# spla-tam/SplaTAM

Measured on AMD Instinct MI355X. Metric: track+map iters/sec @300k Gaussians (render+backward Mpix/s alongside), higher is better.
Workload: dtype f32; 1 GPU; B: 300000 Gaussians, 1200x680, SplaTAM tracking+mapping loop (2:3 mix), isotropic map; fused tracking iterations do not form dL/d(rgb, opacity, scale): the reference computes them, steps them with learning rate 0 and discards the optimizer after the frame (parameters after any number of iterations are identical); mapping iterations take their Adam step on gradients held in registers and do not sto; gaussians=300000, width=1200, height=680, views=8, sync_mode=auto, engine=fused, parallelism=1 process/GPU

## Files before the change

### splatam_amd/csrc/fused.hip

```cpp
#include "splat_device.h"

#include "fused_math.h"

namespace splat {

namespace {

constexpr int kBlock = 256;
constexpr int kFlagSum = SPLAT_ITER_SUMS - 1;

struct FusedArgs {
    SplatCamera cam;
    SplatMap map;
    SplatFrameData frame;
    SplatLossConfig cfg;
    SplatIterWorkspace ws;
    float win[11];
};

__device__ __forceinline__ int c_num_tiles(int W, int H) { return ((W + kTile - 1) / kTile) * ((H + kTile - 1) / kTile); }
__device__ __forceinline__ int c_num_groups(int W, int H) {
    return (((W + kTile - 1) / kTile + SPLAT_GROUP_TILES - 1) / SPLAT_GROUP_TILES) * (((H + kTile - 1) / kTile + SPLAT_GROUP_TILES - 1) / SPLAT_GROUP_TILES);
}

// ... 211 lines not shown
        const uint64_t key = ((uint64_t)dbits[g] << 32) | (uint32_t)i;
        for (int y = y0; y < y1; ++y)
            for (int x = x0; x < x1; ++x) {
                const unsigned tix = (unsigned)(y * c.gx + x);
                const unsigned slot = atomicAdd(&s_tile[tix], 1u);
                if (slot < stride) st.keys[(size_t)tix * stride + slot] = key;
                else spilled = true;
            }
    }
    if (spilled) st.status[1] = 1;
}

__device__ __forceinline__ double *sum_copy(double *sums) {
    const unsigned b = blockIdx.x + gridDim.x * (blockIdx.y + gridDim.y * blockIdx.z);
    return sums + (size_t)(b % SPLAT_ITER_SUM_COPIES) * SPLAT_ITER_SUMS;
}

template <int N>
__device__ __forceinline__ void block_sum_to(double *dst, const float (&v)[N], double *s_part ) {
    const int lane = threadIdx.x & 63, wave = threadIdx.x >> 6, nw = blockDim.x >> 6;
#pragma unroll
    for (int k = 0; k < N; ++k) {
        float x = v[k];
        for (int m = 32; m >= 1; m >>= 1) x += __shfl_xor(x, m, 64);
        if (lane == 0) s_part[k * nw + wave] = (double)x;
    }
    __syncthreads();
    if ((int)threadIdx.x < N) {
        double t = 0.0;
        for (int w = 0; w < nw; ++w) t += s_part[threadIdx.x * nw + w];
        if (t != 0.0) atomicAdd(dst + threadIdx.x, t);
    }
    __syncthreads();
}

__device__ __forceinline__ double sum_total(const double *sums, int k) {
    static_assert(SPLAT_ITER_SUM_COPIES == 64, "one copy per lane");
    double v = sums[(size_t)(threadIdx.x & 63) * SPLAT_ITER_SUMS + k];
    for (int m = 32; m >= 1; m >>= 1) v += __shfl_xor(v, m, 64);
    return v;
}

struct Pixel {
    bool mask;
    float d_err;
    float d_sign;
};

__device__ __forceinline__ float sgn(float x) { return (x > 0.f) ? 1.f : ((x < 0.f) ? -1.f : 0.f); }

__device__ __forceinline__ Pixel depth_pixel(const SplatLossConfig &cfg, float depth, float sil, float depth_sq, float gt, float median) {
    Pixel r;
    const float unc = depth_sq - depth * depth;
    const bool nan_ok = !(depth != depth) && !(unc != unc);
    bool m = gt > 0.f && nan_ok;
    if (cfg.ignore_outlier_depth_loss) m = m && (fabsf(gt - depth) < 10.f * median);
    if (cfg.tracking && cfg.use_sil_for_loss) m = m && (sil > cfg.sil_thres);
    r.mask = m;
    const float diff = gt - depth;
    r.d_err = m ? fabsf(diff) : 0.f;
    r.d_sign = m ? -sgn(diff) : 0.f;
    return r;
}

template <int V>
__global__ __launch_bounds__(kBlock) void track_loss_kernel(FusedArgs a, int HW) {
    __shared__ double s_part[2 * (kBlock / 64)];
    const float *o = a.ws.out6;
    float *g = a.ws.dL_dout6;
    const bool masked_im = a.cfg.use_sil_for_loss || a.cfg.ignore_outlier_depth_loss;
    const float median = a.cfg.ignore_outlier_depth_loss ? a.ws.d_cam[13] : 0.f;
    float acc[2] = {0.f, 0.f};
    const int nvec = HW / V;
    for (int i = blockIdx.x * kBlock + threadIdx.x; i < nvec; i += gridDim.x * kBlock) {
        float in[10][V], out[4][V];
        auto ld = [&](const float *p, float *dst) {
            if constexpr (V == 4) {
                const float4 t = reinterpret_cast<const float4 *>(p)[i];
                dst[0] = t.x; dst[1] = t.y; dst[2] = t.z; dst[3] = t.w;
            } else {
                dst[0] = p[i];
            }
        };
#pragma unroll
        for (int ch = 0; ch < 6; ++ch) ld(o + ch * (size_t)HW, in[ch]);
#pragma unroll
        for (int ch = 0; ch < 3; ++ch) ld(a.frame.im + ch * (size_t)HW, in[6 + ch]);
        ld(a.frame.depth, in[9]);
#pragma unroll
        for (int v = 0; v < V; ++v) {
            const Pixel px = depth_pixel(a.cfg, in[3][v], in[4][v], in[5][v], in[9][v], median);
            acc[0] += px.d_err;
            out[3][v] = a.cfg.use_l1 ? a.cfg.w_depth * px.d_sign : 0.f;
            const bool cm = masked_im ? px.mask : true;
#pragma unroll
            for (int ch = 0; ch < 3; ++ch) {
                const float diff = in[6 + ch][v] - in[ch][v];
                acc[1] += cm ? fabsf(diff) : 0.f;
                out[ch][v] = cm ? -a.cfg.w_im * sgn(diff) : 0.f;
            }
        }
#pragma unroll
        for (int ch = 0; ch < 4; ++ch) {
            if constexpr (V == 4) reinterpret_cast<float4 *>(g + ch * (size_t)HW)[i] = make_float4(out[ch][0], out[ch][1], out[ch][2], out[ch][3]);
            else g[ch * (size_t)HW + i] = out[ch][0];
        }
    }
    block_sum_to<2>(sum_copy(a.ws.sums), acc, s_part);
}

constexpr int kSsimR = 5;
typedef float f2 __attribute__((ext_vector_type(2)));

template <int TW, int TH>
__device__ __forceinline__ bool ssim_tile(int W, int H, int &bx, int &by, int &ch) {
    const int ntx = (W + TW - 1) / TW, nty = (H + TH - 1) / TH, total = 3 * ntx * nty, per = (total + 7) / 8;
    const int b = blockIdx.x, slot = b >> 3, t = (b & 7) * per + slot;
    if (slot >= per || t >= total) return false;
    ch = t / (ntx * nty);
    const int r = t - ch * ntx * nty;
    by = r / ntx;
    bx = r - by * ntx;
    return true;
}

void ssim_window_host(float *g) {
    float s = 0.f;
    for (int k = 0; k < 11; ++k) { g[k] = (float)exp(-(double)((k - 5) * (k - 5)) / 4.5); s += g[k]; }
    for (int k = 0; k < 11; ++k) g[k] /= s;
}

__device__ __forceinline__ float ssim_pixel_dev(float mu1, float mu2, float e11, float e22, float e12, float *dmu1, float *de11, float *de12) {
    const float mu1_sq = mu1 * mu1, mu2_sq = mu2 * mu2, mu12 = mu1 * mu2;
    const float s1 = e11 - mu1_sq, s2 = e22 - mu2_sq, s12 = e12 - mu12;
    const float A = 2.f * mu12 + kSsimC1, B = 2.f * s12 + kSsimC2;
    const float Cd = mu1_sq + mu2_sq + kSsimC1, Dd = s1 + s2 + kSsimC2;
    const float iC = __builtin_amdgcn_rcpf(Cd), iD = __builtin_amdgcn_rcpf(Dd);
    const float iCD = iC * iD;
    const float map = A * B * iCD;
    *dmu1 = (2.f * mu2) * (B - A) * iCD + map * (2.f * mu1) * (iD - iC);
    *de11 = -map * iD;
    *de12 = 2.f * A * iCD;
    return map;
}

// ... 205 lines not shown
            }
#pragma unroll
            for (int j = 0; j < kCR; ++j) { svA[grp * kCR + j][col] = vA[j]; svC[grp * kCR + j][col] = vC[j]; }
        }
    }
    if (tid < kCItems) {
        load_px4<VEC>(a.ws.out6 + ch * HW, y0 + hr, x0 + hc, W, H, own_x);
        load_px4<VEC>(a.frame.im + ch * HW, y0 + hr, x0 + hc, W, H, own_y);
    }
    __syncthreads();
    if (tid >= kCItems) return;
    const float inv_n = 1.0f / (3.0f * (float)HW);
    const float median = a.cfg.ignore_outlier_depth_loss ? a.ws.d_cam[13] : 0.f;
    const float count = s_count;
    f2 oA[4];
    float oC[4];
#pragma unroll
    for (int j = 0; j < 4; ++j) { oA[j] = (f2)(0.f); oC[j] = 0.f; }
#pragma unroll
    for (int t = 0; t < 14; ++t) {
        const f2 pa = svA[hr][hc + t];
        const float pc = svC[hr][hc + t];
#pragma unroll
        for (int j = 0; j < 4; ++j) {
            const int tap = t - j;
            if (tap >= 0 && tap < 11) {
                oA[j] = __builtin_elementwise_fma((f2)(g[tap]), pa, oA[j]);
                oC[j] = fmaf(g[tap], pc, oC[j]);
            }
        }
    }
    float out[4];
#pragma unroll
    for (int j = 0; j < 4; ++j) {
        const float xv = own_x[j], yv = own_y[j];
        const float dssim = oA[j].x + 2.f * xv * oA[j].y + yv * oC[j];
        out[j] = a.cfg.w_im * (0.8f * sgn(xv - yv) * inv_n - 0.2f * inv_n * dssim);
    }
    store_px4<VEC>(a.ws.dL_dout6 + ch * HW, y0 + hr, x0 + hc, W, H, out);
    if (ch == 0) {
        float pre[4][4], dout[4];
        load_px4<VEC>(a.ws.out6 + 3 * HW, y0 + hr, x0 + hc, W, H, pre[0]);
        load_px4<VEC>(a.ws.out6 + 4 * HW, y0 + hr, x0 + hc, W, H, pre[1]);
        load_px4<VEC>(a.ws.out6 + 5 * HW, y0 + hr, x0 + hc, W, H, pre[2]);
        load_px4<VEC>(a.frame.depth, y0 + hr, x0 + hc, W, H, pre[3]);
#pragma unroll
        for (int j = 0; j < 4; ++j) {
            const Pixel px = depth_pixel(a.cfg, pre[0][j], pre[1][j], pre[2][j], pre[3][j], median);
            dout[j] = a.cfg.use_l1 ? a.cfg.w_depth * px.d_sign / count : 0.f;
        }
        store_px4<VEC>(a.ws.dL_dout6 + 3 * HW, y0 + hr, x0 + hc, W, H, dout);
    }
}

struct PoseAdam {
    float *state;
    float beta1, beta2, eps, bc2_sqrt, ss_rot, ss_trans;
};

struct PoseAdamRegs {
    float *pp[7];
    float par[7], m[7], v[7], best;
};

__device__ __forceinline__ void pose_adam_load(const SplatMap &map, int time_idx, const PoseAdam &pa, PoseAdamRegs &r) {
#pragma unroll
    for (int k = 0; k < 7; ++k) {
        r.pp[k] = k < 4 ? map.cam_unnorm_rots + k * map.num_frames + time_idx : map.cam_trans + (k - 4) * map.num_frames + time_idx;
        r.par[k] = *r.pp[k];
        r.m[k] = pa.state[k];
        r.v[k] = pa.state[7 + k];
    }
    r.best = pa.state[14];
}

__device__ __forceinline__ void pose_adam_apply(PoseAdamRegs &r, const float *g, float loss, const PoseAdam &pa) {
    float *state = pa.state;
#pragma unroll
    for (int k = 0; k < 7; ++k)
        r.par[k] = adam_update(r.par[k], g[k], r.m[k], r.v[k], pa.beta1, pa.beta2, k < 4 ? pa.ss_rot : pa.ss_trans, pa.bc2_sqrt, pa.eps);
#pragma unroll
    for (int k = 0; k < 7; ++k) {
        *r.pp[k] = r.par[k];
// ... 300 lines not shown
    else
        hipLaunchKernelGGL((fused_preprocess_kernel<0, kBlock>), dim3((P + kBlock - 1) / kBlock), dim3(kBlock), 0, s, a);
}

hipError_t launch_iter_loss_backward(const SplatCamera &cam, const SplatMap &map, const SplatFrameData &frame,
                                     const SplatLossConfig &cfg, SplatIterWorkspace &ws_in, hipStream_t s, const SplatPoseAdam *pose_adam,
                                     const SplatAdamMap *map_adam) {
    SplatIterWorkspace ws = ws_in;
    if (!group_binning(ws.st, cam)) ws.st.group_stride = 0;
    FusedArgs a{cam, map, frame, cfg, ws, {}};
    ssim_window_host(a.win);
    const int W = cam.image_width, H = cam.image_height, HW = W * H;
    const int T = (int)splat_num_tiles(W, H);
    const int P = map.P;
    hipError_t e = hipSuccess;
    const int gblocks = (P + kBlock - 1) / kBlock;
    launch_fused_preprocess(a, s);
    if (ws.st.tile_stride == 0) {
        e = launch_tile_scan(ws.st, T, s);
        if (e != hipSuccess) return e;
    }
    SplatGaussians g{};
    g.P = P;
    g.channels = 6;
    const bool sort_in_k6 = lists_sorted_by_composite(ws.st);
    e = launch_bin_forward(cam, g, ws.st, s, !sort_in_k6);
    if (e != hipSuccess) return e;
    TrackLossEpilogue ep{frame.im, frame.depth, ws.dL_dout6, ws.sums, cfg.sil_thres, cfg.w_im, cfg.w_depth, cfg.use_sil_for_loss, cfg.use_l1};
    bool loss_done = false;
    const bool fuse_loss = cfg.tracking && !cfg.ignore_outlier_depth_loss;
    if (ws.st.tile_row_end > ws.st.tile_row_begin && !fuse_loss) return hipErrorInvalidValue;
    const bool one_kernel = fuse_loss && sort_in_k6 && cfg.fused_composite != 0;
    const bool full_sums = ws.d_rgb_colors != nullptr || ws.d_logit_opacities != nullptr;
    if (one_kernel) {
        e = launch_render_track_fused(cam, ws.feat8, ws.st, ws.out6, ws.accum, ep, cfg.fused_composite == 2, s, full_sums);
        if (e != hipSuccess) return e;
    } else {
        e = launch_render_forward_feat8(cam, ws.feat8, ws.st, ws.out6, sort_in_k6, s, fuse_loss ? &ep : nullptr, fuse_loss ? &loss_done : nullptr);
        if (e != hipSuccess) return e;
        if (cfg.ignore_outlier_depth_loss) {
            e = launch_depth_error_median(ws.out6, frame.depth, ws.outlier_err, ws.outlier_scratch, HW,
                                          reinterpret_cast<int32_t *>(ws.d_cam) + 9, s);
            if (e != hipSuccess) return e;
        }
        if (cfg.tracking && loss_done) {
        } else if (cfg.tracking) {
            if (HW % 4 == 0) {
                const int blocks = min((HW / 4 + kBlock - 1) / kBlock, 2048);
                hipLaunchKernelGGL(track_loss_kernel<4>, dim3(blocks), dim3(kBlock), 0, s, a, HW);
            } else {
                const int blocks = min((HW + kBlock - 1) / kBlock, 2048);
                hipLaunchKernelGGL(track_loss_kernel<1>, dim3(blocks), dim3(kBlock), 0, s, a, HW);
            }
        } else {
            const int tiles = 3 * ((W + kCW - 1) / kCW) * ((H + kCH - 1) / kCH);
            const dim3 grid(8 * ((tiles + 7) / 8));
            if ((W & 3) == 0 && aligned16(ws.out6) && aligned16(frame.im) && aligned16(frame.depth) && aligned16(ws.ssim_maps) && aligned16(ws.dL_dout6)) {
                hipLaunchKernelGGL(ssim_forward_kernel<true>, grid, dim3(kBlock), 0, s, a, W, H);
                hipLaunchKernelGGL(map_loss_backward_kernel<true>, grid, dim3(kBlock), 0, s, a, W, H);
            } else {
                hipLaunchKernelGGL(ssim_forward_kernel<false>, grid, dim3(kBlock), 0, s, a, W, H);
                hipLaunchKernelGGL(map_loss_backward_kernel<false>, grid, dim3(kBlock), 0, s, a, W, H);
            }
        }
        e = launch_render_backward_feat8(cam, ws.feat8, ws.st, ws.dL_dout6, ws.accum, P, false,
                                         ws.d_rgb_colors != nullptr || (map_adam && map_adam->grad[1]), s,
                                         ws.d_logit_opacities != nullptr || (map_adam && map_adam->grad[3]));
        if (e != hipSuccess) return e;
    }
    PoseAdam pa{};
    if (pose_adam)
        pa = PoseAdam{pose_adam->state, pose_adam->beta1, pose_adam->beta2, pose_adam->eps, pose_adam->bc2_sqrt, pose_adam->step_size_rot,
                      pose_adam->step_size_trans};
    if (P > 0) {
        const bool iso = map.isotropic != 0;
        const bool mapgrads = ws.d_means3D || ws.d_rgb_colors || ws.d_unnorm_rotations || ws.d_logit_opacities || ws.d_log_scales;
        const SplatAdamMap opt = map_adam ? *map_adam : SplatAdamMap{};
        const dim3 grid(gblocks), block(kBlock);
        if (map_adam && iso) hipLaunchKernelGGL((fused_backward_kernel<true, true, true>), grid, block, 0, s, a, opt);
        else if (map_adam) hipLaunchKernelGGL((fused_backward_kernel<true, true, false>), grid, block, 0, s, a, opt);
        else if (mapgrads && iso) hipLaunchKernelGGL((fused_backward_kernel<false, true, true>), grid, block, 0, s, a, opt);
        else if (mapgrads) hipLaunchKernelGGL((fused_backward_kernel<false, true, false>), grid, block, 0, s, a, opt);
        else if (iso) hipLaunchKernelGGL((fused_backward_kernel<false, false, true>), grid, block, 0, s, a, opt);
        else hipLaunchKernelGGL((fused_backward_kernel<false, false, false>), grid, block, 0, s, a, opt);
    }
    if (!cfg.defer_finish) hipLaunchKernelGGL(pose_finish_kernel, dim3(finish_blocks(ws.st)), dim3(256), 0, s, a, HW, pa);
    return hipGetLastError();
}

hipError_t launch_iter_finish(const SplatCamera &cam, const SplatMap &map, const SplatFrameData &frame, const SplatLossConfig &cfg,
                              SplatIterWorkspace &ws, hipStream_t s, const SplatPoseAdam *pose_adam) {
    FusedArgs a{cam, map, frame, cfg, ws, {}};
    PoseAdam pa{};
    if (pose_adam)
        pa = PoseAdam{pose_adam->state, pose_adam->beta1, pose_adam->beta2, pose_adam->eps, pose_adam->bc2_sqrt, pose_adam->step_size_rot,
                      pose_adam->step_size_trans};
    hipLaunchKernelGGL(pose_finish_kernel, dim3(finish_blocks(ws.st)), dim3(256), 0, s, a, cam.image_width * cam.image_height, pa);
    return hipGetLastError();
}

// ... 88 lines not shown
```

### splatam_amd/csrc/render.hip

```cpp
#include <type_traits>

#include "splat_device.h"

#ifndef SPLAT_BLOCK_RADIAL
#define SPLAT_BLOCK_RADIAL 1
#endif

namespace splat {

constexpr int kBatch = 256;
constexpr int kBatchEntries = 255;
constexpr int kSegBytes = 68;
constexpr int kBlockListBytes = 264;


template <int FP>
struct Staged {
    float4 ga;
    float2 mu;
    float feat[FP];
    unsigned mask;
    unsigned id;
    float aux;
};
// ... 939 lines not shown
                const unsigned r2 = rec_of((cur4 >> 16) & 0xFFu);
                load_rec(r2, rb);
                visit(r3, ra);
                const unsigned r1 = rec_of((cur4 >> 8) & 0xFFu);
                load_rec(r1, ra);
                visit(r2, rb);
                const unsigned r0 = rec_of(cur4 & 0xFFu);
                load_rec(r0, rb);
                visit(r1, ra);
                r3 = rec_of(nxt4 >> 24);
                load_rec(r3, ra);
                visit(r0, rb);
                cur4 = nxt4;
            }
        }
        if (nslot > 0) {
            if constexpr ((DBG & 8) == 0) phase2(nslot);
            nslot = 0;
            slot_m = 0xFFull;
            wr_ptr = my_vw + wr_lane;
        }
    }
}

struct BwdArgs {
    SplatCamera cam;
    const float *colors;
    SplatState st;
    const float *dL_dcolor;
    float *accum;
    int T, per_xcd;
    long long *stamps;
};
template <int C, int CS, unsigned DMASK, unsigned SMASK, bool OPAC, bool BG, int DBG = 0>
__device__ __forceinline__ void render_backward_body5(const BwdArgs &args) {
    long long *const stamps = args.stamps;
    long long t_begin = 0;
    if constexpr ((DBG & 1) != 0) t_begin = (long long)wall_clock64();
    auto stamp = [&]() {
        if constexpr ((DBG & 1) != 0)
            if (threadIdx.x == 0 && stamps) { stamps[2 * (size_t)blockIdx.x] = t_begin; stamps[2 * (size_t)blockIdx.x + 1] = (long long)wall_clock64(); }
    };
    constexpr int CL = highest_set_bit(DMASK) + 1;
    static_assert(CL >= 1 && CL <= C, "DMASK names channels of the call");
    constexpr int FP = (CL + 3) / 4 * 4;
    __shared__ Batch<FP> B;
    __shared__ PairBuf PB;
    __shared__ unsigned s_wmax[4];
    const int tile_local = block_tile(args.per_xcd, args.T, launch_order(args.st));
    if (tile_local < 0) { stamp(); return; }
    const BwdArgs &a = args;
    const SplatCamera &cam = a.cam;
    const SplatState &st = a.st;
    const float *const colors = a.colors, *const dL_dcolor = a.dL_dcolor;
    float *const accum = a.accum;
    const int W = cam.image_width, H = cam.image_height;
    const int gx = (W + kTile - 1) / kTile;
    const int tile = tile_local + st.tile_row_begin * gx;
    const int tid = threadIdx.x, lane = tid & 63, wave = tid >> 6;
    const int tx = tile % gx, ty = tile / gx;
    const int px = tx * kTile + (wave & 1) * 8 + (lane & 7), py = ty * kTile + (wave >> 1) * 8 + (lane >> 3);
    const bool inside = px < W && py < H;
    const size_t HW = (size_t)H * W;
    const size_t pix = (size_t)py * W + px;

    const float Tfin = inside ? st.final_T[pix] : 0.f;
    const unsigned last = inside ? (unsigned)st.n_contrib[pix] : 0u;
    float dpix[C], R = 0.f;
#pragma unroll
    for (int ch = 0; ch < C; ++ch) {
        dpix[ch] = 0.f;
        if ((DMASK >> ch) & 1u) {
            dpix[ch] = inside ? dL_dcolor[ch * HW + pix] : 0.f;
            if constexpr (BG) R += Tfin * bg_of(cam, ch) * dpix[ch];
        }
    }
    backward_core<C, CS, DMASK, SMASK, OPAC, DBG>(colors, st, accum, B, PB, s_wmax, tile, tx, ty, tid, inside, Tfin, last, dpix, R, -1);
    stamp();
}

#ifndef SPLAT_K7_MIN_WAVES
#define SPLAT_K7_MIN_WAVES 1
#endif
template <int C, int CS, unsigned DMASK, unsigned SMASK, bool OPAC = true, bool BG = true>
__global__ __launch_bounds__(256, (popcount_c(SMASK) <= 4 ? SPLAT_K7_MIN_WAVES : 1)) void render_backward_kernel5(BwdArgs args) {
    render_backward_body5<C, CS, DMASK, SMASK, OPAC, BG>(args);
}
template <int C, int CS, unsigned DMASK, unsigned SMASK, bool OPAC = true, bool BG = true>
__global__ __launch_bounds__(256, 5) void render_backward_kernel5_w5(BwdArgs args) {
    static_assert(popcount_c(SMASK) <= 2, "the five-wave shape is for the forms whose gradient rows live in registers");
    render_backward_body5<C, CS, DMASK, SMASK, OPAC, BG>(args);
}

struct TrackFusedArgs {
    SplatCamera cam;
    const float *feat8;
    SplatState st;
    float *out6, *accum;
    int T, per_xcd;
    TrackLossEpilogue ep;
};
template <bool KEEP, int DBG, bool FULL>
__device__ __forceinline__ void track_fused_body(const TrackFusedArgs &args) {
    constexpr int C = 6, CS = 8, FP = forward_fp<C, CS, false>();
    using BatchT = Batch<FP, 16, true>;
    constexpr size_t kHead = offsetof(BatchT, vlist);
    constexpr size_t kKeysAt = (kHead + sizeof(BatchT::vlist) + 15) / 16 * 16;
    constexpr size_t kFwd = kKeysAt + sizeof(uint64_t) * (kFusedSortMax + 2);
    constexpr size_t kBwd = (kHead + 15) / 16 * 16 + sizeof(PairBuf);
    __shared__ __attribute__((aligned(16))) unsigned char s_raw[kFwd > kBwd ? kFwd : kBwd];
    __shared__ unsigned s_wmax[4];
    __shared__ double s_loss[2][4];
    BatchT &B = *reinterpret_cast<BatchT *>(s_raw);
    uint64_t *const s_keys = reinterpret_cast<uint64_t *>(s_raw + kKeysAt);
    PairBuf &PB = *reinterpret_cast<PairBuf *>(s_raw + (kHead + 15) / 16 * 16);
    const int tile_local = block_tile(args.per_xcd, args.T, launch_order(args.st));
    if (tile_local < 0) return;
    const TrackFusedArgs &a = args;
    const SplatCamera &cam = a.cam;
// ... 238 lines not shown
            default: hipLaunchKernelGGL((render_track_fused_kernel<false>), dim3(8 * per), dim3(256), 0, s, TrackFusedArgs{cam, feat8, st, out6, accum, T, per, ep}); break;
        }
        return hipGetLastError();
    }
    if (full_sums) {
        if (keep_planes) hipLaunchKernelGGL((render_track_fused_full_kernel<true>), dim3(8 * per), dim3(256), 0, s, TrackFusedArgs{cam, feat8, st, out6, accum, T, per, ep});
        else hipLaunchKernelGGL((render_track_fused_full_kernel<false>), dim3(8 * per), dim3(256), 0, s, TrackFusedArgs{cam, feat8, st, out6, accum, T, per, ep});
        return hipGetLastError();
    }
    if (keep_planes) {
        auto k = render_track_fused_kernel<true>;
        hipLaunchKernelGGL(k, dim3(8 * per), dim3(256), 0, s, TrackFusedArgs{cam, feat8, st, out6, accum, T, per, ep});
    } else {
        auto k = render_track_fused_kernel<false>;
        hipLaunchKernelGGL(k, dim3(8 * per), dim3(256), 0, s, TrackFusedArgs{cam, feat8, st, out6, accum, T, per, ep});
    }
    return hipGetLastError();
}

hipError_t launch_render_backward_feat8(const SplatCamera &cam, const float *feat8, const SplatState &st, const float *dL_dout6,
                                        float *accum, int P, bool zero_accum, bool rgb_sums, hipStream_t s, bool opacity_sum) {
    const int T = launch_tiles(cam, st);
    if (zero_accum) {
        hipError_t e = hipMemsetAsync(accum, 0, sizeof(float) * SPLAT_GRAD_STRIDE * (size_t)P, s);
        if (e != hipSuccess) return e;
    }
    if (T == 0 || P == 0) return hipSuccess;
    if (rgb_sums) launch_bwd<6, 8, 0xFu, 0xFu, true, false>(cam, feat8, st, dL_dout6, accum, T, s);
    else if (opacity_sum) launch_bwd<6, 8, 0xFu, 0x8u, true, false>(cam, feat8, st, dL_dout6, accum, T, s);
    else launch_bwd<6, 8, 0xFu, 0x8u, false, false>(cam, feat8, st, dL_dout6, accum, T, s);
    return hipGetLastError();
}

hipError_t launch_render_backward_rgb_only(const SplatCamera &cam, const float *feat8, const SplatState &st, const float *dL_dout6,
                                           float *accum, int P, hipStream_t s) {
    const int T = launch_tiles(cam, st);
    if (T == 0 || P == 0) return hipSuccess;
    const int per = (T + 7) / 8;
    hipLaunchKernelGGL((render_backward_kernel5_w5<6, 8, 0x7u, 0x0u, false, false>), dim3(8 * per), dim3(256), 0, s, BwdArgs{cam, feat8, st, dL_dout6, accum, T, per, nullptr});
    return hipGetLastError();
}

}
```

### splatam_amd/csrc/splat_device.h

```cpp
#pragma once

#include <hip/hip_runtime.h>

#include "../../include/splat_hip.h"
#include "splat_math.h"

namespace splat {

constexpr int kWave = 64;

hipError_t launch_preprocess_forward(const SplatCamera &cam, const SplatGaussians &g, SplatState &st, hipStream_t s);
hipError_t launch_tile_count_reset(SplatState &st, int T, hipStream_t s);
hipError_t launch_tile_scan(SplatState &st, int T, hipStream_t s);
hipError_t launch_bin_forward(const SplatCamera &cam, const SplatGaussians &g, SplatState &st, hipStream_t s, bool sort = true,
                              bool counted_per_workgroup = false);

constexpr int kDenseThreads = 1024, kDenseGaussians = 4096, kDenseMaxTilesLds = 12 * 1024;
inline bool dense_exact_lists(const SplatState &st, int P, int T) {
    return st.tile_stride == 0 && st.sub_bins > 1 && P >= 8 * kDenseGaussians && T <= kDenseMaxTilesLds;
}
inline bool lists_sorted_by_composite(const SplatState &st) { return st.max_list_hint > 0 && st.max_list_hint + st.max_list_hint / 4 <= 1024; }
inline bool group_binning(const SplatState &st, int W, int H) {
    const int gx = (W + SPLAT_TILE - 1) / SPLAT_TILE, gy = (H + SPLAT_TILE - 1) / SPLAT_TILE;
    const int groups = ((gx + SPLAT_GROUP_TILES - 1) / SPLAT_GROUP_TILES) * ((gy + SPLAT_GROUP_TILES - 1) / SPLAT_GROUP_TILES);
    return st.group_stride > 0 && st.group_count && st.group_recs && st.tile_stride > 0 && lists_sorted_by_composite(st) && groups <= 8192;
}
hipError_t launch_render_forward(const SplatCamera &cam, const SplatGaussians &g, SplatState &st,
                                 float *out_color, float *out_depth, hipStream_t s);
hipError_t launch_render_backward(const SplatCamera &cam, const SplatGaussians &g, const SplatState &st,
                                  SplatGrads &gr, hipStream_t s);
hipError_t launch_preprocess_backward(const SplatCamera &cam, const SplatGaussians &g, const SplatState &st,
                                      SplatGrads &gr, hipStream_t s);
hipError_t launch_mark_visible(int P, const float *means3D, const float *view, uint8_t *present, hipStream_t s);
hipError_t launch_same_geometry(int P, const float *oa, const float *ob, const float *sa, const float *sb, const float *ra, const float *rb,
                                int *differ, hipStream_t s);
struct TrackLossEpilogue {
    const float *im;
    const float *depth;
    float *dL_dout6;
    double *sums;
    float sil_thres, w_im, w_depth;
    int use_sil_for_loss, use_l1;
};
hipError_t launch_render_forward_feat8(const SplatCamera &cam, const float *feat8, SplatState &st, float *out6, bool sort_in_kernel,
                                       hipStream_t s, const TrackLossEpilogue *ep = nullptr, bool *ep_done = nullptr);
hipError_t launch_render_track_fused(const SplatCamera &cam, const float *feat8, SplatState &st, float *out6, float *accum,
                                     const TrackLossEpilogue &ep, bool keep_planes, hipStream_t s, bool full_sums = false);
hipError_t launch_render_backward_feat8(const SplatCamera &cam, const float *feat8, const SplatState &st, const float *dL_dout6,
                                        float *accum, int P, bool zero_accum, bool rgb_sums, hipStream_t s, bool opacity_sum = true);
hipError_t launch_iter_loss_backward(const SplatCamera &cam, const SplatMap &map, const SplatFrameData &frame,
                                     const SplatLossConfig &cfg, SplatIterWorkspace &ws, hipStream_t s, const SplatPoseAdam *pose_adam = nullptr,
                                     const SplatAdamMap *map_adam = nullptr);
hipError_t launch_iter_finish(const SplatCamera &cam, const SplatMap &map, const SplatFrameData &frame, const SplatLossConfig &cfg,
                              SplatIterWorkspace &ws, hipStream_t s, const SplatPoseAdam *pose_adam);
hipError_t launch_iter_adam_map(const SplatMap &map, const SplatAdamMap &opt, hipStream_t s);
hipError_t launch_iter_fold_sums(double *sums, hipStream_t s);
hipError_t launch_iter_adam_pose(const SplatMap &map, int time_idx, const float *d_cam, float *state, float beta1, float beta2,
                                 float eps, float bc2_sqrt, float ss_rot, float ss_trans, hipStream_t s);
hipError_t launch_iter_render(const SplatCamera &cam, const SplatMap &map, const SplatFrameData &frame, SplatIterWorkspace &ws,
                              hipStream_t s);
hipError_t launch_map_add(const SplatMapStore &st, const SplatAddArgs &a, hipStream_t s);
hipError_t launch_map_prune(const SplatMapStore &st, const SplatPruneArgs &a, hipStream_t s);
hipError_t launch_map_densify_select(const SplatMapStore &st, const SplatDensifyArgs &a, hipStream_t s);
hipError_t launch_map_duplicate(const SplatMapStore &st, const SplatDensifyArgs &a, hipStream_t s);
hipError_t launch_iter_means2d_accumulate(const SplatCamera &cam, const SplatMap &map, SplatIterWorkspace &ws, float *accum, float *denom,
                                          float *means2D_grad, hipStream_t s);
hipError_t launch_render_backward_rgb_only(const SplatCamera &cam, const float *feat8, const SplatState &st, const float *dL_dout6,
                                           float *accum, int P, hipStream_t s);
size_t map_scratch_words(long long n);
int map_row_floats(const SplatMapStore &st);
extern int g_debug_skip_count;
extern int g_debug_k7_bits;
extern long long *g_debug_stamps;
hipError_t launch_selftest(int which, const void *in, void *out, int n, hipStream_t s);

#if defined(__HIPCC__)

__device__ __forceinline__ void load_cam(CamConst &c, const SplatCamera &cam) {
    init_cam(c, cam.viewmatrix, cam.projmatrix, cam.image_width, cam.image_height, cam.tanfovx, cam.tanfovy,
             cam.scale_modifier);
}

// ... 454 lines not shown
    const int t0 = band * per_xcd, t1 = min(T, t0 + per_xcd);
    if (tid == 0) *s_max = 1u;
    s_hist[tid] = 0u;
    __syncthreads();
    unsigned mx = 0u;
    for (int t = t0 + tid; t < t1; t += 256) mx = max(mx, work[t]);
    mx = wave_max_u32(mx);
    if ((tid & 63) == 0) atomicMax(s_max, mx);
    __syncthreads();
    const float scale = 255.0f / (float)*s_max;
    for (int t = t0 + tid; t < t1; t += 256) atomicAdd(&s_hist[255 - (int)((float)work[t] * scale)], 1u);
    __syncthreads();
    if (tid < 64) {
        unsigned c[4], sum = 0u;
#pragma unroll
        for (int k = 0; k < 4; ++k) { c[k] = s_hist[4 * tid + k]; sum += c[k]; }
        unsigned incl = sum;
        for (int d = 1; d < 64; d <<= 1) {
            const unsigned o = (unsigned)__shfl_up((int)incl, d, 64);
            if (tid >= d) incl += o;
        }
        unsigned run = incl - sum;
#pragma unroll
        for (int k = 0; k < 4; ++k) { s_off[4 * tid + k] = run; run += c[k]; }
    }
    __syncthreads();
    for (int t = t0 + tid; t < t1; t += 256) {
        const unsigned pos = atomicAdd(&s_off[255 - (int)((float)work[t] * scale)], 1u);
        order[t0 + pos] = (uint32_t)t + 1u;
    }
    for (int t = max(t1, t0) + tid; t < t0 + per_xcd; t += 256) order[t] = 0xFFFFFFFFu;
}

#endif

}
```

### splatam_amd/fused.py

```python
from __future__ import annotations

import ctypes as C
import os
import math

import torch

from . import _capi
from .rasterizer import _cached_contiguous

PARAM_ORDER = ("means3D", "rgb_colors", "unnorm_rotations", "logit_opacities", "log_scales")
VARIABLE_KEYS = ("max_2D_radius", "means2D_gradient_accum", "denom", "timestep")
_FLAG_SLOTS = 16


class FusedEngine:
    def __init__(self, params, cam, capacity=None, track_max_radius=None, gaussian_capacity=None, variables=None, row_headroom=0.0):
        self.L = _capi.lib()
        self.params = params
        self.variables = variables
        self.cam_settings = cam
        dev = params['means3D'].device
        if dev.type != "cuda":
            raise RuntimeError("FusedEngine needs CUDA/HIP tensors; the HIP library has no CPU path")
# ... 27 lines not shown
        self.num_groups = (((W + 15) // 16 + GT - 1) // GT) * (((H + 15) // 16 + GT - 1) // GT)
        self.tile_order_on = os.environ.get("SPLAT_TILE_ORDER", "1") != "0"
        self.order_per_view = os.environ.get("SPLAT_TILE_ORDER_PER_VIEW", "1") != "0"
        self._natural_order, self._orders = torch.zeros_like(b['tile_order']), {}
        b['pose_state'] = torch.zeros(_capi.SPLAT_POSE_STATE, dtype=f32, **z)
        self.max_2D_radius = self.store['max_2D_radius'] if self.managed else track_max_radius
        b['counts'] = torch.zeros(8, dtype=i32, **z)
        self._widths = [3, 3, 4, 1, 1 if self.iso else 3]
        self._grad_store = torch.zeros(_FLAG_SLOTS + sum(self._widths) * P_alloc, dtype=f32, **z)
        self._m_store = {k: torch.zeros(P_alloc, w, dtype=f32, **z) for k, w in zip(PARAM_ORDER, self._widths)}
        self._v_store = {k: torch.zeros(P_alloc, w, dtype=f32, **z) for k, w in zip(PARAM_ORDER, self._widths)}
        self._layout_rows()
        self.map_step = 0
        self.pose_step = 0
        self.track_time_idx = None
        self.max_list_hint = 0
        self.tile_stride = 0
        self.num_tiles = T
        self.allow_buckets = True
        self.group_bins = True
        self.fused_adam_max_rows = int(os.environ.get("SPLAT_FUSED_ADAM_MAX_ROWS", 1 << 30))
        self._tile_rows = None
        self._stats_partial = False
        self.sub_bins = 1
        self.creation_order = bool(self.managed and P == 0)
        self.keep_map_grads = True
        self.use_recs = {"0": 0, "1": 1}.get(os.environ.get("SPLAT_TILE_RECS", "auto"), 2)
        self._alloc_lists(self.capacity)
        self._cam = self._make_cam(cam)
        self._cam_ok = {}
        self._frame_keep = None
        self.track_fused = os.environ.get("SPLAT_TRACK_FUSED", "1") != "0"
        self.track_fused_full = os.environ.get("SPLAT_TRACK_FUSED_FULL", "1") != "0"
        self.fold_sums = os.environ.get("SPLAT_FOLD_SUMS", "1") != "0"
        self.skipped_iterations = 0
        self._learnt_P = None

    _ROW_ARRAYS = (("st.conic_opacity", "conic", torch.float32, (4,)), ("st.xy", "xy", torch.float32, (2,)), ("st.rect", "rect", torch.int32, (2,)),
                   ("st.depth", "depth", torch.float32, ()), ("st.radii", "radii", torch.int32, ()), ("feat8", "feat8", torch.float32, (8,)),
                   ("accum", "accum", torch.float32, (_capi.SPLAT_GRAD_STRIDE,)))
    _FIXED_ARRAYS = (("st.tile_count", "tile_count", torch.int32), ("st.tile_base", "tile_base", torch.int32),
                     ("st.tile_cursor", "tile_cursor", torch.int32), ("st.long_base", "long_base", torch.int32),
                     ("st.group_count", "group_count", torch.int32), ("st.status", "status", torch.int32),
                     ("st.tile_work", "tile_work", torch.int32), ("st.tile_order", "tile_order", torch.int32),
                     ("st.final_T", "final_T", torch.float32),
                     ("st.n_contrib", "n_contrib", torch.int32), ("out6", "out6", torch.float32), ("dL_dout6", "dL_dout6", torch.float32),
                     ("ssim_maps", "ssim_maps", torch.float32), ("sums", "sums", torch.float64), ("d_cam", "d_cam", torch.float32))

    def _layout(self, rows, capacity=0, group_stride=0, outlier=False):
        flags = _capi.SPLAT_LAYOUT_SSIM | _capi.SPLAT_LAYOUT_TILE_ORDER | _capi.SPLAT_LAYOUT_RECS | (_capi.SPLAT_LAYOUT_OUTLIER if outlier else 0)
        return _capi.iter_workspace_layout(int(rows), self.W, self.H, int(capacity), int(group_stride), flags)

    def _new(self, lay, name, dtype, tail=()):
        n = lay.bytes[name] // torch.empty((), dtype=dtype).element_size()
        t = (torch.zeros if lay.zero_init[name] else torch.empty)(n, dtype=dtype, device=self.dev)
        return t.view((-1,) + tuple(tail)) if tail else t

    def _alloc_fixed(self, lay):
        for name, key, dtype in self._FIXED_ARRAYS:
            self.buf[key] = self._new(lay, name, dtype)
        H, W = self.H, self.W
        for key, lead in (('final_T', ()), ('n_contrib', ()), ('out6', (6,)), ('dL_dout6', (6,)), ('ssim_maps', (9,))):
            self.buf[key] = self.buf[key].view(lead + (H, W))

    def _alloc_rows(self, lay):
        for name, key, dtype, tail in self._ROW_ARRAYS:
# ... 453 lines not shown
                self._orders.pop(next(iter(self._orders)))
            o = self._natural_order.clone()
        self._orders[view] = o
        self.buf['tile_order'] = o

    def _stream(self):
        return torch.cuda.current_stream(self.dev).cuda_stream

    @staticmethod
    def loss_config(cfg, tracking, do_ba=False, defer_finish=False, fused_composite=0):
        c = _capi.SplatLossConfig()
        c.defer_finish = int(defer_finish)
        c.fused_composite = int(fused_composite)
        c.tracking = int(tracking)
        c.camera_grad = int(tracking or do_ba)
        c.gaussians_grad = int(not tracking)
        c.use_sil_for_loss, c.sil_thres = int(cfg['use_sil_for_loss']), float(cfg['sil_thres'])
        c.use_l1, c.ignore_outlier_depth_loss = int(cfg['use_l1']), int(cfg['ignore_outlier_depth_loss'])
        c.w_im, c.w_depth = float(cfg['loss_weights']['im']), float(cfg['loss_weights']['depth'])
        return c

    def loss_backward(self, curr_data, time_idx, cfg, tracking, map_grads=None, do_ba=False, pose_adam=None, map_adam=None,
                      tile_rows=None, keep_planes=None):
        if map_grads is None:
            map_grads = not tracking
        self._check_cam(curr_data)
        fr = _capi.SplatFrameData()
        im, depth = curr_data['im'], curr_data['depth']
        w2c = curr_data['w2c']
        if not (im.is_contiguous() and depth.is_contiguous() and w2c.is_contiguous()):
            im, depth, w2c = im.contiguous(), depth.contiguous(), w2c.contiguous()
        fr.im, fr.depth, fr.w2c, fr.time_idx = im.data_ptr(), depth.data_ptr(), w2c.data_ptr(), int(time_idx)
        self._frame_keep = (im, depth, w2c)
        if keep_planes is None:
            keep_planes = pose_adam is None
        full_ok = self.track_fused_full and 0 < self.max_list_hint <= 400
        one_kernel = (2 if keep_planes else 1) if (tracking and self.track_fused and (not map_grads or full_ok)) else 0
        lc = self.loss_config(cfg, tracking, do_ba, defer_finish=tile_rows is not None, fused_composite=one_kernel)
        self._tile_rows = tile_rows
        self._stats_partial = tile_rows is not None
        self._lc_keep = lc
        if lc.ignore_outlier_depth_loss and 'outlier_err' not in self.buf:
            lay = self._layout(0, outlier=True)
            self.buf['outlier_err'] = self._new(lay, "outlier_err", torch.float32)
            self.buf['outlier_scratch'] = self._new(lay, "outlier_scratch", torch.int32)
        self._select_order(int(time_idx))
        ws = self._workspace(map_grads, with_ssim=not tracking)
        m = self._map_struct()
        with torch.cuda.device(self.dev):
            if pose_adam is not None:
                _capi.check(self.L.splat_iter_tracking_step(C.byref(self._cam), C.byref(m), C.byref(fr), C.byref(lc), C.byref(ws),
                                                            C.byref(pose_adam), self._stream()), "splat_iter_tracking_step")
            elif map_adam is not None:
                _capi.check(self.L.splat_iter_mapping_step(C.byref(self._cam), C.byref(m), C.byref(fr), C.byref(lc), C.byref(ws),
                                                           C.byref(map_adam), self._stream()), "splat_iter_mapping_step")
            else:
                _capi.check(self.L.splat_iter_loss_backward(C.byref(self._cam), C.byref(m), C.byref(fr), C.byref(lc), C.byref(ws),
                                                            self._stream()), "splat_iter_loss_backward")
        self._tile_rows = None
        self._fr_keep = fr

    def finish_iteration(self, pose_adam=None):
        ws = self._workspace(False, with_ssim=False)
        m = self._map_struct()
        with torch.cuda.device(self.dev):
            _capi.check(self.L.splat_iter_finish(C.byref(self._cam), C.byref(m), C.byref(self._fr_keep), C.byref(self._lc_keep), C.byref(ws),
                                                 C.byref(pose_adam) if pose_adam is not None else None, self._stream()), "splat_iter_finish")

    def tile_row_band(self, rank, world):
        from .dist import tile_row_band
# ... 184 lines not shown
```

Measured before the change: 4364 iters/s.

## Fuse mapping loss backward (SSIM/L1 gradient) into render backward kernel prologue

For mapping iterations, the separate map_loss_backward kernel is dropped. Its per-pixel dL/d(rgb, depth) computation, including the separable SSIM window pass, now runs as a prologue inside the render backward kernel, with the pair buffer in LDS reused as scratch. This avoids one kernel launch and a full write and read of the dL_dout6 planes, unless the planes must be kept. In exchange the prologue adds extra LDS traffic, a barrier and register pressure to an already heavy backward kernel.

```diff
diff --git a/splatam_amd/csrc/fused.hip b/splatam_amd/csrc/fused.hip
--- a/splatam_amd/csrc/fused.hip
+++ b/splatam_amd/csrc/fused.hip
@@ -267,35 +267,6 @@
         if (t != 0.0) atomicAdd(dst + threadIdx.x, t);
     }
     __syncthreads();
-}
-
-__device__ __forceinline__ double sum_total(const double *sums, int k) {
-    static_assert(SPLAT_ITER_SUM_COPIES == 64, "one copy per lane");
-    double v = sums[(size_t)(threadIdx.x & 63) * SPLAT_ITER_SUMS + k];
-    for (int m = 32; m >= 1; m >>= 1) v += __shfl_xor(v, m, 64);
-    return v;
-}
-
-struct Pixel {
-    bool mask;
-    float d_err;
-    float d_sign;
-};
-
-__device__ __forceinline__ float sgn(float x) { return (x > 0.f) ? 1.f : ((x < 0.f) ? -1.f : 0.f); }
-
-__device__ __forceinline__ Pixel depth_pixel(const SplatLossConfig &cfg, float depth, float sil, float depth_sq, float gt, float median) {
-    Pixel r;
-    const float unc = depth_sq - depth * depth;
-    const bool nan_ok = !(depth != depth) && !(unc != unc);
-    bool m = gt > 0.f && nan_ok;
-    if (cfg.ignore_outlier_depth_loss) m = m && (fabsf(gt - depth) < 10.f * median);
-    if (cfg.tracking && cfg.use_sil_for_loss) m = m && (sil > cfg.sil_thres);
-    r.mask = m;
-    const float diff = gt - depth;
-    r.d_err = m ? fabsf(diff) : 0.f;
-    r.d_sign = m ? -sgn(diff) : 0.f;
-    return r;
 }
 
 template <int V>
@@ -345,7 +316,6 @@
 }
 
 constexpr int kSsimR = 5;
-typedef float f2 __attribute__((ext_vector_type(2)));
 
 template <int TW, int TH>
 __device__ __forceinline__ bool ssim_tile(int W, int H, int &bx, int &by, int &ch) {
@@ -617,11 +587,7 @@
     }
     float out[4];
 #pragma unroll
-    for (int j = 0; j < 4; ++j) {
-        const float xv = own_x[j], yv = own_y[j];
-        const float dssim = oA[j].x + 2.f * xv * oA[j].y + yv * oC[j];
-        out[j] = a.cfg.w_im * (0.8f * sgn(xv - yv) * inv_n - 0.2f * inv_n * dssim);
-    }
+    for (int j = 0; j < 4; ++j) out[j] = map_dl_dcolor(oA[j].x, oA[j].y, oC[j], own_x[j], own_y[j], a.cfg.w_im, inv_n);
     store_px4<VEC>(a.ws.dL_dout6 + ch * HW, y0 + hr, x0 + hc, W, H, out);
     if (ch == 0) {
         float pre[4][4], dout[4];
@@ -630,10 +596,7 @@
         load_px4<VEC>(a.ws.out6 + 5 * HW, y0 + hr, x0 + hc, W, H, pre[2]);
         load_px4<VEC>(a.frame.depth, y0 + hr, x0 + hc, W, H, pre[3]);
 #pragma unroll
-        for (int j = 0; j < 4; ++j) {
-            const Pixel px = depth_pixel(a.cfg, pre[0][j], pre[1][j], pre[2][j], pre[3][j], median);
-            dout[j] = a.cfg.use_l1 ? a.cfg.w_depth * px.d_sign / count : 0.f;
-        }
+        for (int j = 0; j < 4; ++j) dout[j] = map_dl_ddepth(a.cfg, pre[0][j], pre[1][j], pre[2][j], pre[3][j], median, count);
         store_px4<VEC>(a.ws.dL_dout6 + 3 * HW, y0 + hr, x0 + hc, W, H, dout);
     }
 }
@@ -1000,6 +963,9 @@
     if (ws.st.tile_row_end > ws.st.tile_row_begin && !fuse_loss) return hipErrorInvalidValue;
     const bool one_kernel = fuse_loss && sort_in_k6 && cfg.fused_composite != 0;
     const bool full_sums = ws.d_rgb_colors != nullptr || ws.d_logit_opacities != nullptr;
+    const bool rgb_sums = ws.d_rgb_colors != nullptr || (map_adam && map_adam->grad[1]);
+    const bool opacity_sum = ws.d_logit_opacities != nullptr || (map_adam && map_adam->grad[3]);
+    const bool map_loss_in_k7 = !cfg.tracking && cfg.fused_composite != 0 && !cfg.ignore_outlier_depth_loss && rgb_sums;
     if (one_kernel) {
         e = launch_render_track_fused(cam, ws.feat8, ws.st, ws.out6, ws.accum, ep, cfg.fused_composite == 2, s, full_sums);
         if (e != hipSuccess) return e;
@@ -1025,15 +991,19 @@
             const dim3 grid(8 * ((tiles + 7) / 8));
             if ((W & 3) == 0 && aligned16(ws.out6) && aligned16(frame.im) && aligned16(frame.depth) && aligned16(ws.ssim_maps) && aligned16(ws.dL_dout6)) {
                 hipLaunchKernelGGL(ssim_forward_kernel<true>, grid, dim3(kBlock), 0, s, a, W, H);
-                hipLaunchKernelGGL(map_loss_backward_kernel<true>, grid, dim3(kBlock), 0, s, a, W, H);
+                if (!map_loss_in_k7) hipLaunchKernelGGL(map_loss_backward_kernel<true>, grid, dim3(kBlock), 0, s, a, W, H);
             } else {
                 hipLaunchKernelGGL(ssim_forward_kernel<false>, grid, dim3(kBlock), 0, s, a, W, H);
-                hipLaunchKernelGGL(map_loss_backward_kernel<false>, grid, dim3(kBlock), 0, s, a, W, H);
-            }
-        }
-        e = launch_render_backward_feat8(cam, ws.feat8, ws.st, ws.dL_dout6, ws.accum, P, false,
-                                         ws.d_rgb_colors != nullptr || (map_adam && map_adam->grad[1]), s,
-                                         ws.d_logit_opacities != nullptr || (map_adam && map_adam->grad[3]));
+                if (!map_loss_in_k7) hipLaunchKernelGGL(map_loss_backward_kernel<false>, grid, dim3(kBlock), 0, s, a, W, H);
+            }
+        }
+        if (map_loss_in_k7) {
+            MapLossPrologue lp{ws.ssim_maps, ws.out6, frame.im, frame.depth, ws.sums, cfg.fused_composite == 2 ? ws.dL_dout6 : nullptr, cfg, {}};
+            for (int k = 0; k < 11; ++k) lp.win[k] = a.win[k];
+            e = launch_render_backward_map_loss(cam, ws.feat8, ws.st, lp, ws.accum, P, s);
+        } else {
+            e = launch_render_backward_feat8(cam, ws.feat8, ws.st, ws.dL_dout6, ws.accum, P, false, rgb_sums, s, opacity_sum);
+        }
         if (e != hipSuccess) return e;
     }
     PoseAdam pa{};
diff --git a/splatam_amd/csrc/render.hip b/splatam_amd/csrc/render.hip
--- a/splatam_amd/csrc/render.hip
+++ b/splatam_amd/csrc/render.hip
@@ -995,8 +995,8 @@
     int T, per_xcd;
     long long *stamps;
 };
-template <int C, int CS, unsigned DMASK, unsigned SMASK, bool OPAC, bool BG, int DBG = 0>
-__device__ __forceinline__ void render_backward_body5(const BwdArgs &args) {
+template <int C, int CS, unsigned DMASK, unsigned SMASK, bool OPAC, bool BG, int DBG = 0, bool LOSS = false>
+__device__ __forceinline__ void render_backward_body5(const BwdArgs &args, const MapLossPrologue *lp = nullptr) {
     long long *const stamps = args.stamps;
     long long t_begin = 0;
     if constexpr ((DBG & 1) != 0) t_begin = (long long)wall_clock64();
@@ -1034,9 +1034,14 @@
     for (int ch = 0; ch < C; ++ch) {
         dpix[ch] = 0.f;
         if ((DMASK >> ch) & 1u) {
-            dpix[ch] = inside ? dL_dcolor[ch * HW + pix] : 0.f;
+            dpix[ch] = inside && !LOSS ? dL_dcolor[ch * HW + pix] : 0.f;
             if constexpr (BG) R += Tfin * bg_of(cam, ch) * dpix[ch];
         }
+    }
+    if constexpr (LOSS) {
+        static_assert(!BG && DMASK == 0xFu, "the mapping iteration's form: zero background, gradient in r, g, b, depth");
+        static_assert(sizeof(MapLossLds) <= sizeof(PairBuf), "the prologue borrows the pair buffer");
+        map_loss_prologue<C>(*lp, *reinterpret_cast<MapLossLds *>(&PB), W, H, tx, ty, tid, px, py, inside, dpix);
     }
     backward_core<C, CS, DMASK, SMASK, OPAC, DBG>(colors, st, accum, B, PB, s_wmax, tile, tx, ty, tid, inside, Tfin, last, dpix, R, -1);
     stamp();
@@ -1048,6 +1053,10 @@
 template <int C, int CS, unsigned DMASK, unsigned SMASK, bool OPAC = true, bool BG = true>
 __global__ __launch_bounds__(256, (popcount_c(SMASK) <= 4 ? SPLAT_K7_MIN_WAVES : 1)) void render_backward_kernel5(BwdArgs args) {
     render_backward_body5<C, CS, DMASK, SMASK, OPAC, BG>(args);
+}
+template <int C, int CS, unsigned DMASK, unsigned SMASK, bool OPAC = true>
+__global__ __launch_bounds__(256, (popcount_c(SMASK) <= 4 ? SPLAT_K7_MIN_WAVES : 1)) void render_backward_map_loss_kernel5(BwdArgs args, MapLossPrologue lp) {
+    render_backward_body5<C, CS, DMASK, SMASK, OPAC, false, 0, true>(args, &lp);
 }
 template <int C, int CS, unsigned DMASK, unsigned SMASK, bool OPAC = true, bool BG = true>
 __global__ __launch_bounds__(256, 5) void render_backward_kernel5_w5(BwdArgs args) {
@@ -1352,6 +1361,16 @@
     return hipGetLastError();
 }
 
+hipError_t launch_render_backward_map_loss(const SplatCamera &cam, const float *feat8, const SplatState &st, const MapLossPrologue &lp,
+                                           float *accum, int P, hipStream_t s) {
+    const int T = launch_tiles(cam, st);
+    if (T == 0 || P == 0) return hipSuccess;
+    const int per = (T + 7) / 8;
+    hipLaunchKernelGGL((render_backward_map_loss_kernel5<6, 8, 0xFu, 0xFu, true>), dim3(8 * per), dim3(256), 0, s,
+                       BwdArgs{cam, feat8, st, lp.dL_dout6, accum, T, per, nullptr}, lp);
+    return hipGetLastError();
+}
+
 hipError_t launch_render_backward_rgb_only(const SplatCamera &cam, const float *feat8, const SplatState &st, const float *dL_dout6,
                                            float *accum, int P, hipStream_t s) {
     const int T = launch_tiles(cam, st);
diff --git a/splatam_amd/csrc/splat_device.h b/splatam_amd/csrc/splat_device.h
--- a/splatam_amd/csrc/splat_device.h
+++ b/splatam_amd/csrc/splat_device.h
@@ -48,6 +48,18 @@
                                      const TrackLossEpilogue &ep, bool keep_planes, hipStream_t s, bool full_sums = false);
 hipError_t launch_render_backward_feat8(const SplatCamera &cam, const float *feat8, const SplatState &st, const float *dL_dout6,
                                         float *accum, int P, bool zero_accum, bool rgb_sums, hipStream_t s, bool opacity_sum = true);
+struct MapLossPrologue {
+    const float *ssim_maps;
+    const float *out6;
+    const float *im;
+    const float *depth;
+    const double *sums;
+    float *dL_dout6;
+    SplatLossConfig cfg;
+    float win[11];
+};
+hipError_t launch_render_backward_map_loss(const SplatCamera &cam, const float *feat8, const SplatState &st, const MapLossPrologue &lp,
+                                           float *accum, int P, hipStream_t s);
 hipError_t launch_iter_loss_backward(const SplatCamera &cam, const SplatMap &map, const SplatFrameData &frame,
                                      const SplatLossConfig &cfg, SplatIterWorkspace &ws, hipStream_t s, const SplatPoseAdam *pose_adam = nullptr,
                                      const SplatAdamMap *map_adam = nullptr);
@@ -568,6 +580,151 @@
     for (int t = max(t1, t0) + tid; t < t0 + per_xcd; t += 256) order[t] = 0xFFFFFFFFu;
 }
 
+__device__ __forceinline__ double sum_total(const double *sums, int k) {
+    static_assert(SPLAT_ITER_SUM_COPIES == 64, "one copy per lane");
+    double v = sums[(size_t)(threadIdx.x & 63) * SPLAT_ITER_SUMS + k];
+    for (int m = 32; m >= 1; m >>= 1) v += __shfl_xor(v, m, 64);
+    return v;
+}
+
+struct Pixel {
+    bool mask;
+    float d_err;
+    float d_sign;
+};
+
+__device__ __forceinline__ float sgn(float x) { return (x > 0.f) ? 1.f : ((x < 0.f) ? -1.f : 0.f); }
+
+__device__ __forceinline__ Pixel depth_pixel(const SplatLossConfig &cfg, float depth, float sil, float depth_sq, float gt, float median) {
+    Pixel r;
+    const float unc = depth_sq - depth * depth;
+    const bool nan_ok = !(depth != depth) && !(unc != unc);
+    bool m = gt > 0.f && nan_ok;
+    if (cfg.ignore_outlier_depth_loss) m = m && (fabsf(gt - depth) < 10.f * median);
+    if (cfg.tracking && cfg.use_sil_for_loss) m = m && (sil > cfg.sil_thres);
+    r.mask = m;
+    const float diff = gt - depth;
+    r.d_err = m ? fabsf(diff) : 0.f;
+    r.d_sign = m ? -sgn(diff) : 0.f;
+    return r;
+}
+
+__device__ __forceinline__ float map_dl_dcolor(float oAx, float oAy, float oC, float xv, float yv, float w_im, float inv_n) {
+    const float dssim = oAx + 2.f * xv * oAy + yv * oC;
+    return w_im * (0.8f * sgn(xv - yv) * inv_n - 0.2f * inv_n * dssim);
+}
+
+__device__ __forceinline__ float map_dl_ddepth(const SplatLossConfig &cfg, float depth, float sil, float depth_sq, float gt, float median, float count) {
+    const Pixel px = depth_pixel(cfg, depth, sil, depth_sq, gt, median);
+    return cfg.use_l1 ? cfg.w_depth * px.d_sign / count : 0.f;
+}
+
+typedef float f2 __attribute__((ext_vector_type(2)));
+
+constexpr int kMlR = 5;
+constexpr int kMlCols = kTile + 2 * kMlR;
+constexpr int kMlRows = 2;
+constexpr int kMlGroups = kTile / kMlRows;
+constexpr int kMlStride = kMlCols + 1;
+struct MapLossLds {
+    f2 a[3][kTile][kMlStride];
+    float c[3][kTile][kMlStride];
+};
+static_assert(kMlCols * kMlGroups <= 256, "one trip of the vertical pass");
+
+template <int C>
+__device__ __forceinline__ void map_loss_prologue(const MapLossPrologue &lp, MapLossLds &L, const int W, const int H, const int tx, const int ty,
+                                                  const int tid, const int px, const int py, const bool inside, float (&dpix)[C]) {
+    static_assert(C >= 4, "r, g, b, depth");
+    float g[11];
+#pragma unroll
+    for (int k = 0; k < 11; ++k) g[k] = lp.win[k];
+    const size_t HW = (size_t)H * W;
+    const size_t own = (size_t)min(py, H - 1) * W + min(px, W - 1);
+    float xo[3], yo[3], pre[4];
+#pragma unroll
+    for (int ch = 0; ch < 3; ++ch) { xo[ch] = lp.out6[ch * HW + own]; yo[ch] = lp.im[ch * HW + own]; }
+#pragma unroll
+    for (int k = 0; k < 3; ++k) pre[k] = lp.out6[(3 + k) * HW + own];
+    pre[3] = lp.depth[own];
+    const float count = (float)sum_total(lp.sums, 2);
+    {
+        const int grp = tid / kMlCols, col = tid - grp * kMlCols;
+        if (grp < kMlGroups) {
+            const int xx = tx * kTile - kMlR + col;
+            const bool cin = xx >= 0 && xx < W;
+            const int xc = min(max(xx, 0), W - 1);
+            unsigned off[kMlRows + 10], in_rows = 0u;
+#pragma unroll
+            for (int t = 0; t < kMlRows + 10; ++t) {
+                const int yy = ty * kTile + grp * kMlRows - kMlR + t;
+                off[t] = 4u * (unsigned)(min(max(yy, 0), H - 1) * W + xc);
+                if (cin && yy >= 0 && yy < H) in_rows |= 1u << t;
+            }
+            const char *const M0 = reinterpret_cast<const char *>(lp.ssim_maps);
+            const char *const M1 = reinterpret_cast<const char *>(lp.ssim_maps + HW), *const M2 = reinterpret_cast<const char *>(lp.ssim_maps + 2 * HW);
+#pragma unroll 1
+            for (int ch = 0; ch < 3; ++ch) {
+                const unsigned cb = (unsigned)(12 * HW) * (unsigned)ch;
+                float v0[kMlRows + 10], v1[kMlRows + 10], v2[kMlRows + 10];
+#pragma unroll
+                for (int t = 0; t < kMlRows + 10; ++t) {
+                    const unsigned o = off[t] + cb;
+                    v0[t] = *reinterpret_cast<const float *>(M0 + o);
+                    v1[t] = *reinterpret_cast<const float *>(M1 + o);
+                    v2[t] = *reinterpret_cast<const float *>(M2 + o);
+                }
+                asm volatile("" ::: "memory");
+#pragma unroll
+                for (int t = 0; t < kMlRows + 10; ++t) {
+                    const bool in = (in_rows >> t) & 1u;
+                    v0[t] = in ? v0[t] : 0.f;
+                    v1[t] = in ? v1[t] : 0.f;
+                    v2[t] = in ? v2[t] : 0.f;
+                }
+                f2 vA[kMlRows];
+                float vC[kMlRows];
+#pragma unroll
+                for (int j = 0; j < kMlRows; ++j) { vA[j] = (f2)(0.f); vC[j] = 0.f; }
+#pragma unroll
+                for (int t = 0; t < kMlRows + 10; ++t) {
+                    const f2 p = {v0[t], v1[t]};
+#pragma unroll
+                    for (int j = 0; j < kMlRows; ++j) {
+                        const int tap = t - j;
+                        if (tap >= 0 && tap < 11) {
+                            vA[j] = __builtin_elementwise_fma((f2)(g[tap]), p, vA[j]);
+                            vC[j] = fmaf(g[tap], v2[t], vC[j]);
+                        }
+                    }
+                }
+#pragma unroll
+                for (int j = 0; j < kMlRows; ++j) { L.a[ch][grp * kMlRows + j][col] = vA[j]; L.c[ch][grp * kMlRows + j][col] = vC[j]; }
+            }
+        }
+    }
+    __syncthreads();
+    const int r = py - ty * kTile, c = px - tx * kTile;
+    const float inv_n = 1.0f / (3.0f * (float)HW);
+    const size_t pix = (size_t)py * W + px;
+#pragma unroll
+    for (int ch = 0; ch < 3; ++ch) {
+        f2 oA = (f2)(0.f);
+        float oC = 0.f;
+#pragma unroll
+        for (int tap = 0; tap < 11; ++tap) {
+            oA = __builtin_elementwise_fma((f2)(g[tap]), L.a[ch][r][c + tap], oA);
+            oC = fmaf(g[tap], L.c[ch][r][c + tap], oC);
+        }
+        dpix[ch] = inside ? map_dl_dcolor(oA.x, oA.y, oC, xo[ch], yo[ch], lp.cfg.w_im, inv_n) : 0.f;
+        if (lp.dL_dout6 && inside) lp.dL_dout6[ch * HW + pix] = dpix[ch];
+    }
+    dpix[3] = inside ? map_dl_ddepth(lp.cfg, pre[0], pre[1], pre[2], pre[3], 0.f, count) : 0.f;
+    if (lp.dL_dout6 && inside) lp.dL_dout6[3 * HW + pix] = dpix[3];
+#pragma unroll
+    for (int ch = 4; ch < C; ++ch) dpix[ch] = 0.f;
+}
+
 #endif
 
 }
diff --git a/splatam_amd/fused.py b/splatam_amd/fused.py
--- a/splatam_amd/fused.py
+++ b/splatam_amd/fused.py
@@ -83,6 +83,7 @@
         self._frame_keep = None
         self.track_fused = os.environ.get("SPLAT_TRACK_FUSED", "1") != "0"
         self.track_fused_full = os.environ.get("SPLAT_TRACK_FUSED_FULL", "1") != "0"
+        self.map_loss_in_k7 = os.environ.get("SPLAT_MAP_LOSS_IN_K7", "1") != "0"
         self.fold_sums = os.environ.get("SPLAT_FOLD_SUMS", "1") != "0"
         self.skipped_iterations = 0
         self._learnt_P = None
@@ -602,10 +603,13 @@
             im, depth, w2c = im.contiguous(), depth.contiguous(), w2c.contiguous()
         fr.im, fr.depth, fr.w2c, fr.time_idx = im.data_ptr(), depth.data_ptr(), w2c.data_ptr(), int(time_idx)
         self._frame_keep = (im, depth, w2c)
+        map_planes = map_adam is None or bool(keep_planes)
         if keep_planes is None:
             keep_planes = pose_adam is None
         full_ok = self.track_fused_full and 0 < self.max_list_hint <= 400
         one_kernel = (2 if keep_planes else 1) if (tracking and self.track_fused and (not map_grads or full_ok)) else 0
+        if not tracking and self.map_loss_in_k7:
+            one_kernel = 2 if map_planes else 1
         lc = self.loss_config(cfg, tracking, do_ba, defer_finish=tile_rows is not None, fused_composite=one_kernel)
         self._tile_rows = tile_rows
         self._stats_partial = tile_rows is not None
```

Result: faster. 4424 iters/s (median of 6 runs) (+1.4%).
